# miguelmartin75/txt2vid

Hardware: AMD Instinct MI355X
Metric: TGANv2 GAN train throughput (G+D steps x global batch), 16x64x64 videos/sec (higher is better)
Workload: dtype f32; 1 GPU; BASELINE configs[1]: unconditional TGANv2 16x64x64x1, per-GPU batch 32, fp32, RSGAN + GP 0.5, Adam 2e-4 (0.5,0.999), 1 D + 1 G step, subsample_input pyramid 8/16/32/64; global_batch=32, per_gpu_batch=32, parallelism=dp1

## Files before the change

include/t2v_hip.h:

```cpp
#ifndef T2V_HIP_H
#define T2V_HIP_H

#include <stdint.h>

#ifdef __cplusplus
extern "C" {
#endif

#define T2V_OK 0
#define T2V_EINVAL (-1)
#define T2V_ELAUNCH (-2)

#define T2V_MAX_TAPS 27

typedef struct {
    int32_t N, Cin, D, H, W, Cout;
    int32_t ntaps;
    int8_t dz[T2V_MAX_TAPS], dy[T2V_MAX_TAPS], dx[T2V_MAX_TAPS];
    int8_t pad_[3];
} t2v_conv_geom;

#define T2V_MAX_GROUPS 8
typedef struct {
    const float* x;
    float* y;
    const float* mask;
    int32_t N, D, H, W;
    int32_t ntaps;
    int32_t dstride;
    int32_t ydstride;
    int32_t yoff, Dy;
    int8_t dz[T2V_MAX_TAPS], dy[T2V_MAX_TAPS], dx[T2V_MAX_TAPS], widx[T2V_MAX_TAPS];
} t2v_conv_group;

#define T2V_CONV_BIAS 1
#define T2V_CONV_RELU_IN 2
#define T2V_CONV_ACCUM 4
#define T2V_CONV_ACCUM_BIAS 16
#define T2V_CONV_BF16 32
#define T2V_CONV_MASK_OUT 8

int t2v_pack_weight(const float* w, float* wp, int Cout, int Cin, int T, const int32_t* taps, int ntaps,
                    int mode, void* stream);

int t2v_pack_weight_into(const float* w, float* wp, int Cout, int Cin, int T, const int32_t* taps, int ntaps,
                         int mode, int dst_rows, int dst_cols, int row_off, int col_off, void* stream);

typedef struct {
    const float* src;
    float* dst;
    int32_t Cout, Cin, T, ntaps, mode, dst_rows, dst_cols, row_off, col_off;
    int32_t block_begin;
    int32_t bx, by;
    int8_t taps[T2V_MAX_TAPS];
    int8_t pad_[5];
} t2v_pack_job;
int t2v_pack_job_bytes(void);
int t2v_pack_multi(const void* table , int njobs, int total_blocks, void* stream);

int t2v_conv_fwd(const float* x, const float* wp, const float* bias, float* y, float* ws, const t2v_conv_geom* g,
                 int flags, void* stream);
int64_t t2v_conv_fwd_ws_floats(const t2v_conv_geom* g);

int64_t t2v_conv_wgrad_slab_floats(const t2v_conv_geom* g, int T);
int t2v_conv_wgrad(const float* x, const float* gy, float* dw, float* slab, const t2v_conv_geom* g,
                   const int32_t* taps, int T, int flags, void* stream);

int64_t t2v_conv_fwd_grouped_ws_floats(const t2v_conv_group* groups, int ngroups, int Cin, int Cout);
int t2v_conv_fwd_grouped(const t2v_conv_group* groups, int ngroups, int Cin, int Cout, const float* wp,
                         const float* bias, float* ws, int flags, void* stream);
int64_t t2v_conv_wgrad_grouped_slab_floats(const t2v_conv_group* groups, int ngroups, int Cin, int Cout, int kD,
                                           int kH, int kW);
int t2v_conv_wgrad_grouped(const t2v_conv_group* groups, int ngroups, int Cin, int Cout, int kD, int kH, int kW,
                           float* dw, float* slab, int flags, void* stream);
#define T2V_WGRAD_MAX_SRC 6
typedef struct {
    const float* slab;
    const float* bias_slab;
    int32_t ntaps, S;
    int8_t map[T2V_MAX_TAPS];
    int8_t pad_[5];
    int64_t tap_stride;
    int64_t split_stride;
} t2v_wgrad_src;
typedef struct {
    float* dw;
    float* dbias;
    int64_t CoCi;
    int32_t T, Cout, nsrc;
    int32_t accum, accum_bias;
    int32_t kind;
    int32_t block_begin, nblocks;
    int32_t tap_major;
    int32_t pad_;
    t2v_wgrad_src src[T2V_WGRAD_MAX_SRC];
} t2v_wgrad_dest;
int t2v_conv_wgrad_grouped_partial(const t2v_conv_group* groups, int ngroups, int Cin, int Cout, int kD, int kH, int kW,
                                   float* slab, int want_bias, int flags, t2v_wgrad_src* out_src, void* stream);
int t2v_wgrad_dest_bytes(void);
int t2v_wgrad_reduce_multi(const void* table , int ndest, int total_blocks, void* stream);

int t2v_conv_fwd_plan(const t2v_conv_group* groups, int ngroups, int Cin, int Cout, int flags, int32_t* out);
int t2v_conv_wgrad_plan(const t2v_conv_group* groups, int ngroups, int Cin, int Cout, int kD, int kH, int kW, int32_t* out);
int64_t t2v_conv_wgrad_grouped_bias_slab_floats(const t2v_conv_group* groups, int ngroups, int Cin, int Cout, int kD,
                                                int kH, int kW);
int t2v_conv_wgrad_grouped_bias(const t2v_conv_group* groups, int ngroups, int Cin, int Cout, int kD, int kH, int kW,
                                float* dw, float* dbias, float* slab, int flags, void* stream);

int t2v_pack_weight_bf16(const float* w, void* wpb, int Cout, int Cin, int T, const int32_t* taps, int ntaps, int mode, void* stream);
int t2v_conv_fwd_grouped_bf16_ok(const t2v_conv_group* groups, int ngroups, int Cin, int Cout);
// ... 314 lines not shown
```

txt2vid_amd/_lib.py:

```python
import ctypes as C
import os

_HERE = os.path.dirname(os.path.abspath(__file__))
LIB_PATH = os.environ.get('T2V_LIB') or os.path.join(_HERE, 'csrc', 'libt2v_hip.so')

MAX_TAPS = 27


class ConvGeom(C.Structure):
    _fields_ = [('N', C.c_int32), ('Cin', C.c_int32), ('D', C.c_int32), ('H', C.c_int32), ('W', C.c_int32),
                ('Cout', C.c_int32), ('ntaps', C.c_int32),
                ('dz', C.c_int8 * MAX_TAPS), ('dy', C.c_int8 * MAX_TAPS), ('dx', C.c_int8 * MAX_TAPS),
                ('pad_', C.c_int8 * 3)]


class ConvGroup(C.Structure):
    _fields_ = [('x', C.c_void_p), ('y', C.c_void_p), ('mask', C.c_void_p), ('N', C.c_int32), ('D', C.c_int32), ('H', C.c_int32), ('W', C.c_int32),
                ('ntaps', C.c_int32), ('dstride', C.c_int32), ('ydstride', C.c_int32), ('yoff', C.c_int32), ('Dy', C.c_int32),
                ('dz', C.c_int8 * MAX_TAPS), ('dy', C.c_int8 * MAX_TAPS), ('dx', C.c_int8 * MAX_TAPS), ('widx', C.c_int8 * MAX_TAPS)]


class AdamJob(C.Structure):
    _fields_ = [('p', C.c_void_p), ('g', C.c_void_p), ('m', C.c_void_p), ('v', C.c_void_p), ('n', C.c_int64)]

# ... 34 lines not shown


WGRAD_MAX_SRC = 6


class WgradSrc(C.Structure):
    _fields_ = [('slab', C.c_void_p), ('bias_slab', C.c_void_p), ('ntaps', C.c_int32), ('S', C.c_int32),
                ('map', C.c_int8 * MAX_TAPS), ('pad_', C.c_int8 * 5), ('tap_stride', C.c_int64), ('split_stride', C.c_int64)]


class WgradDest(C.Structure):
    _fields_ = [('dw', C.c_void_p), ('dbias', C.c_void_p), ('CoCi', C.c_int64), ('T', C.c_int32), ('Cout', C.c_int32),
                ('nsrc', C.c_int32), ('accum', C.c_int32), ('accum_bias', C.c_int32), ('kind', C.c_int32),
                ('block_begin', C.c_int32), ('nblocks', C.c_int32), ('tap_major', C.c_int32), ('pad_', C.c_int32),
                ('src', WgradSrc * WGRAD_MAX_SRC)]


class AugMember(C.Structure):
    _fields_ = [('x', C.c_void_p), ('y', C.c_void_p), ('u', C.c_void_p), ('N', C.c_int32), ('C', C.c_int32), ('T', C.c_int32),
                ('S', C.c_int32), ('row_stride', C.c_int32), ('rows', C.c_int32), ('policy', C.c_int32), ('reserved', C.c_int32)]


class AdaLevel(C.Structure):
    _fields_ = [('real', C.c_void_p), ('fake', C.c_void_p), ('count', C.c_int32), ('reserved', C.c_int32)]


class LecamGrad(C.Structure):
    _fields_ = [('real', C.c_void_p), ('fake', C.c_void_p), ('d_real', C.c_void_p), ('d_fake', C.c_void_p), ('count', C.c_int32),
                ('reserved', C.c_int32)]


class ProjMember(C.Structure):
    _fields_ = [('g', C.c_void_p), ('f', C.c_void_p), ('s', C.c_void_p), ('base', C.c_void_p), ('out', C.c_void_p), ('b', C.c_int32),
                ('reserved', C.c_int32)]


class MbstdMember(C.Structure):
    _fields_ = [('f', C.c_void_p), ('g', C.c_void_p * 2), ('base', C.c_void_p * 2), ('gam', C.c_void_p), ('y', C.c_void_p * 2),
                ('stat', C.c_void_p), ('out', C.c_void_p), ('b', C.c_int32), ('seg', C.c_int32)]


MAX_GROUPS = 8
_P = C.c_void_p
_I = C.c_int
_L = C.c_int64
_F = C.c_float
_I3 = C.POINTER(C.c_int32)
_G = C.POINTER(ConvGeom)

SIGNATURES = {
    't2v_pack_weight': [_P, _P, _I, _I, _I, _I3, _I, _I, _P],
    't2v_pack_job_bytes': [],
    't2v_pack_multi': [_P, _I, _I, _P],
    't2v_pack_weight_into': [_P, _P, _I, _I, _I, _I3, _I, _I, _I, _I, _I, _I, _P],
    't2v_conv_fwd': [_P, _P, _P, _P, _P, _G, _I, _P],
    't2v_conv_fwd_ws_floats': [_G],
    't2v_conv_wgrad_slab_floats': [_G, _I],
    't2v_conv_fwd_grouped_ws_floats': [_P, _I, _I, _I],
    't2v_conv_fwd_grouped': [_P, _I, _I, _I, _P, _P, _P, _I, _P],
    't2v_conv_wgrad_grouped_slab_floats': [_P, _I, _I, _I, _I, _I, _I],
    't2v_conv_fwd_plan': [_P, _I, _I, _I, _I, _I3],
    't2v_nonlocal_ok': [_I, _I],
    't2v_nonlocal_fwd': [_P, _P, _P, _P, _P, _I, _I, _I, _I, _I, _P],
    't2v_nonlocal_bwd': [_P, _P, _P, _P, _P, _P, _P, _P, _P, _P, _I, _I, _I, _I, _I, _P],
    't2v_conv_wgrad_grouped_partial': [_P, _I, _I, _I, _I, _I, _I, _P, _I, _I, _P, _P],
    't2v_wgrad_dest_bytes': [],
    't2v_wgrad_reduce_multi': [_P, _I, _I, _P],
    't2v_conv_wgrad_plan': [_P, _I, _I, _I, _I, _I, _I, _I3],
    't2v_pack_weight_bf16': [_P, _P, _I, _I, _I, _P, _I, _I, _P],
    't2v_conv_fwd_grouped_bf16_ok': [_P, _I, _I, _I],
    't2v_conv_fwd_bf16_plan': [_P, _I, _I, _I, _I, _I3],
    't2v_conv_fwd_grouped_bf16': [_P, _I, _I, _I, _P, _P, _P, _I, _P],
    't2v_conv_wgrad_grouped': [_P, _I, _I, _I, _I, _I, _I, _P, _P, _I, _P],
    't2v_conv_wgrad_grouped_bias_slab_floats': [_P, _I, _I, _I, _I, _I, _I],
    't2v_conv_wgrad_grouped_bias': [_P, _I, _I, _I, _I, _I, _I, _P, _P, _P, _I, _P],
    't2v_conv_wgrad': [_P, _P, _P, _P, _G, _I3, _I, _I, _P],
    't2v_channel_sum_ws_floats': [_I, _I, _L],
    't2v_channel_sum': [_P, _P, _P, _I, _I, _L, _I, _P],
    't2v_channel_sum_grouped_ws_floats': [_P, _I, _I],
    't2v_channel_sum_grouped': [_P, _I, _I, _P, _P, _I, _P],
    't2v_relu': [_P, _P, _L, _P],
    't2v_relu_mask': [_P, _P, _P, _L, _P],
    't2v_add': [_P, _P, _P, _L, _P],
    't2v_axpby': [_F, _P, _F, _P, _P, _L, _P],
    't2v_fill': [_P, _F, _L, _P],
    't2v_tanh': [_P, _P, _L, _P],
    't2v_tanh_bwd': [_P, _P, _P, _L, _P],
    't2v_avgpool3d': [_P, _P, _P, _I, _I, _I, _I, _I, _I, _I, _I3, _I3, _I3, _P],
    't2v_avgpool3d_bwd': [_P, _P, _I, _I, _I, _I, _I, _I, _I, _I3, _I3, _I3, _P],
    't2v_avgpool3d_multi': [_P, _I, _P],
    't2v_avgpool3d_bwd_multi': [_P, _I, _P],
    't2v_rowsum': [_P, _P, _L, _L, _P],
    't2v_rowbcast': [_P, _P, _L, _L, _P],
    't2v_upsample2x': [_P, _P, _L, _I, _I, _P],
    't2v_upsample2x_bwd': [_P, _P, _L, _I, _I, _P],
    't2v_upsample2x_add': [_P, _P, _P, _L, _I, _I, _P],
    't2v_rsgan_mean_multi': [_P, _I, _P, _P],
    't2v_rsgan_mean_multi_bwd': [_P, _I, _P, _P],
    't2v_bn_ws_floats': [_I, _I, _L],
    't2v_bn_plan': [_I, _I, _L, _I3],
    't2v_bn_stats': [_P, _P, _P, _P, _P, _I, _I, _L, _F, _F, _P],
    't2v_bn_apply': [_P, _P, _P, _P, _P, _I, _I, _L, _I, _P],
    't2v_bn_bwd': [_P, _P, _P, _P, _P, _P, _P, _P, _P, _I, _I, _L, _I, _P],
    't2v_bn_train_fwd': [_P, _P, _P, _P, _P, _P, _P, _P, _I, _I, _L, _F, _F, _I, _P, _P],
    't2v_bn_train_bwd': [_P, _P, _P, _P, _P, _P, _P, _P, _P, _I, _I, _L, _I, _P],
    't2v_bn_train_fwd_up': [_P, _P, _P, _P, _P, _P, _P, _P, _I, _I, _I, _I, _F, _F, _I, _P, _P],
# ... 134 lines not shown
```

txt2vid_amd/csrc/conv.hip:

```cpp
#include <hip/hip_runtime.h>
#include <stdint.h>
#include "../../include/t2v_hip.h"

typedef float f32x16 __attribute__((ext_vector_type(16)));

#ifdef T2V_STAMPS
__device__ unsigned long long* g_stamps = nullptr;
__device__ unsigned int g_stamps_cap = 0;
extern "C" int t2v_stamps_set(void* buf, unsigned int cap_records) {
    if (hipMemcpyToSymbol(HIP_SYMBOL(g_stamps), &buf, sizeof(buf)) != hipSuccess) return -1;
    if (hipMemcpyToSymbol(HIP_SYMBOL(g_stamps_cap), &cap_records, sizeof(cap_records)) != hipSuccess) return -1;
    return 0;
}
__device__ __forceinline__ unsigned long long stamp_now() {
    unsigned long long t;
    __builtin_amdgcn_sched_barrier(0);
    asm volatile("s_memtime %0\n\ts_waitcnt lgkmcnt(0)" : "=s"(t) :: "memory");
    __builtin_amdgcn_sched_barrier(0);
    return t;
}
#define STAMP(v) const unsigned long long v = stamp_now()
#define STAMP_ACC(acc, a, b) acc += (b) - (a)
#else
#define STAMP(v)
// ... 48 lines not shown
            g_prof_cur = r;
        }
    }
    ~ProfScope() { g_prof_cur = nullptr; }
    static void set_plan(const int32_t* plan, int n) {
        if (g_prof_cur) for (int i = 0; i < n && i < 8; ++i) g_prof_cur->plan[i] = plan[i];
    }
};
#define T2V_LAUNCH_PROF(kernel, grid, block, shm, stream, ...) do {                                                      \
        (void)hipGetLastError();                                                                                          \
        if (g_prof_cur) {                                                                                                 \
            ProfRec* r_ = g_prof_cur; g_prof_cur = nullptr;                                                               \
            hipExtLaunchKernelGGL(kernel, grid, block, shm, stream, r_->e0, r_->e1, 0, __VA_ARGS__);                      \
        } else hipLaunchKernelGGL(kernel, grid, block, shm, stream, __VA_ARGS__);                                         \
    } while (0)

extern "C" int t2v_prof_begin(int max_records) {
    if (max_records < 1 || max_records > (1 << 20)) return T2V_EINVAL;
    if ((int)g_prof.recs.size() < max_records) {
        size_t old = g_prof.recs.size();
        g_prof.recs.resize(max_records);
        for (size_t i = old; i < g_prof.recs.size(); ++i) {
            if (hipEventCreate(&g_prof.recs[i].e0) != hipSuccess || hipEventCreate(&g_prof.recs[i].e1) != hipSuccess) return T2V_ELAUNCH;
        }
    }
    g_prof.used = 0;
    g_prof.on = true;
    return T2V_OK;
}
extern "C" int t2v_prof_end(double* out, int nkinds) {
    g_prof.on = false;
    if (!out || nkinds < 1) return T2V_EINVAL;
    for (int i = 0; i < nkinds * 3; ++i) out[i] = 0.0;
    FILE* dump = nullptr;
    if (const char* path = getenv("T2V_PROF_DUMP")) dump = fopen(path, "w");
    if (dump) fprintf(dump, "kind,flops,ms,M,Cin,Cout,taps,groups,S,plan\n");
    for (size_t i = 0; i < g_prof.used; ++i) {
        ProfRec& r = g_prof.recs[i];
        if (hipEventSynchronize(r.e1) != hipSuccess) return T2V_ELAUNCH;
        float ms = 0.f;
        if (hipEventElapsedTime(&ms, r.e0, r.e1) != hipSuccess) return T2V_ELAUNCH;
        if (r.kind >= 0 && r.kind < nkinds) { out[r.kind * 3] += ms; out[r.kind * 3 + 1] += r.flops; out[r.kind * 3 + 2] += 1.0; }
        if (dump) fprintf(dump, "%d,%.0f,%.6f,%ld,%d,%d,%d,%d,%d,%d:%d:%d:%d:%d:%d:%d:%d\n", r.kind, r.flops, ms, r.M, r.Cin, r.Cout, r.taps,
                          r.groups, r.S, r.plan[0], r.plan[1], r.plan[2], r.plan[3], r.plan[4], r.plan[5], r.plan[6], r.plan[7]);
    }
    if (dump) fclose(dump);
    int dropped = (g_prof.used >= g_prof.recs.size()) ? 1 : 0;
    g_prof.used = 0;
    return dropped;
}

struct TapList { int32_t n; int32_t t[T2V_MAX_TAPS]; };

__global__ __launch_bounds__(256) void pack_weight_kernel(const float* __restrict__ w, float* __restrict__ wp,
                                                          int Cout, int Cin, int T, TapList taps, int mode, int dst_rows,
                                                          int dst_cols, int row_off, int col_off) {
    __shared__ float tile[32][33];
    const int j = blockIdx.z;
    const bool src_tm = mode & 8;
    mode &= 7;
    const int t = mode ? (T - 1 - taps.t[j]) : taps.t[j];
    const int tx = threadIdx.x & 31, ty = threadIdx.x >> 5;
    const int co0 = blockIdx.y * 32, ci0 = blockIdx.x * 32;
    const size_t sco = src_tm ? (size_t)Cin : (size_t)Cin * T, sci = src_tm ? 1 : (size_t)T;
    const size_t st = src_tm ? (size_t)t * Cout * Cin : (size_t)t;
    if (mode == 0) {
        for (int r = ty; r < 32; r += 8) {
            int co = co0 + r, ci = ci0 + tx;
            tile[r][tx] = (co < Cout && ci < Cin) ? w[co * sco + ci * sci + st] : 0.f;
        }
        __syncthreads();
        for (int r = ty; r < 32; r += 8) {
            int ci = ci0 + r, co = co0 + tx;
            if (ci < Cin && co < Cout) wp[((size_t)j * dst_rows + row_off + ci) * dst_cols + col_off + co] = tile[tx][r];
        }
    } else {
        for (int r = ty; r < 32; r += 8) {
            int co = co0 + r, ci = ci0 + tx;
            if (co < Cout && ci < Cin)
                wp[((size_t)j * dst_rows + row_off + co) * dst_cols + col_off + ci] = w[co * sco + ci * sci + st];
        }
    }
}

extern "C" int t2v_pack_weight_into(const float* w, float* wp, int Cout, int Cin, int T, const int32_t* taps, int ntaps,
                                    int mode, int dst_rows, int dst_cols, int row_off, int col_off, void* stream) {
    if (!w || !wp || ntaps < 1 || ntaps > T2V_MAX_TAPS || T > T2V_MAX_TAPS || row_off < 0 || col_off < 0) return T2V_EINVAL;
    if ((mode & ~8) != 0 && (mode & ~8) != 1) return T2V_EINVAL;
    const int rows = (mode & 7) ? Cout : Cin, cols = (mode & 7) ? Cin : Cout;
    if (row_off + rows > dst_rows || col_off + cols > dst_cols) return T2V_EINVAL;
    TapList tl;
    tl.n = ntaps;
    for (int i = 0; i < ntaps; ++i) {
        if (taps[i] < 0 || taps[i] >= T) return T2V_EINVAL;
        tl.t[i] = taps[i];
    }
    dim3 grid((Cin + 31) / 32, (Cout + 31) / 32, ntaps);
    T2V_LAUNCH(pack_weight_kernel, grid, dim3(256), 0, (hipStream_t)stream, w, wp, Cout, Cin, T, tl, mode, dst_rows, dst_cols,
               row_off, col_off);
    return launch_status();
}

extern "C" int t2v_pack_weight(const float* w, float* wp, int Cout, int Cin, int T, const int32_t* taps, int ntaps,
                               int mode, void* stream) {
    return t2v_pack_weight_into(w, wp, Cout, Cin, T, taps, ntaps, mode, (mode & 7) ? Cout : Cin, (mode & 7) ? Cin : Cout, 0, 0, stream);
}


struct PackJob {
    const float* src;
    float* dst;
    int32_t Cout, Cin, T, ntaps, mode, dst_rows, dst_cols, row_off, col_off, block_begin, bx, by;
    int8_t taps[T2V_MAX_TAPS];
    int8_t pad_[5];
};

__global__ __launch_bounds__(256) void pack_multi_kernel(const PackJob* __restrict__ table, int njobs) {
    __shared__ float tile[32][33];
    __shared__ PackJob job;
    if (threadIdx.x == 0) {
        int lo = 0, hi = njobs - 1;
        while (lo < hi) {
            const int mid = (lo + hi + 1) >> 1;
            if (table[mid].block_begin <= (int)blockIdx.x) lo = mid; else hi = mid - 1;
        }
        job = table[lo];
    }
    __syncthreads();
    const int b = (int)blockIdx.x - job.block_begin;
    const int bxi = b % job.bx, byi = (b / job.bx) % job.by, j = b / (job.bx * job.by);
    const int Cout = job.Cout, Cin = job.Cin, T = job.T;
    const int jm = job.mode & 7;
    const bool src_tm = job.mode & 8;
    const bool mirror = jm == 1 || jm == 3, transpose = jm == 0 || jm == 3, b16 = jm >= 2;
    const int t = mirror ? (T - 1 - job.taps[j]) : job.taps[j];
    const size_t sco = src_tm ? (size_t)Cin : (size_t)Cin * T, sci = src_tm ? 1 : (size_t)T;
    const size_t st = src_tm ? (size_t)t * Cout * Cin : (size_t)t;
    const int tx = threadIdx.x & 31, ty = threadIdx.x >> 5;
    const int co0 = byi * 32, ci0 = bxi * 32;
    const float* __restrict__ w = job.src;
    float* __restrict__ wp = job.dst;
    __bf16* __restrict__ wpb = reinterpret_cast<__bf16*>(job.dst);
    if (transpose) {
        for (int r = ty; r < 32; r += 8) {
            int co = co0 + r, ci = ci0 + tx;
            tile[r][tx] = (co < Cout && ci < Cin) ? w[co * sco + ci * sci + st] : 0.f;
        }
        __syncthreads();
        for (int r = ty; r < 32; r += 8) {
            int ci = ci0 + r, co = co0 + tx;
            if (ci < Cin && co < Cout) {
                const size_t o = ((size_t)j * job.dst_rows + job.row_off + ci) * job.dst_cols + job.col_off + co;
                if (b16) wpb[o] = (__bf16)tile[tx][r]; else wp[o] = tile[tx][r];
            }
        }
    } else {
        for (int r = ty; r < 32; r += 8) {
            int co = co0 + r, ci = ci0 + tx;
            if (co < Cout && ci < Cin) {
                const size_t o = ((size_t)j * job.dst_rows + job.row_off + co) * job.dst_cols + job.col_off + ci;
                const float v = w[co * sco + ci * sci + st];
                if (b16) wpb[o] = (__bf16)v; else wp[o] = v;
            }
        }
    }
}

extern "C" int t2v_pack_job_bytes(void) { return (int)sizeof(PackJob); }

extern "C" int t2v_pack_multi(const void* table, int njobs, int total_blocks, void* stream) {
    if (!table || njobs < 1 || total_blocks < 1) return T2V_EINVAL;
    T2V_LAUNCH(pack_multi_kernel, dim3((unsigned)total_blocks), dim3(256), 0, (hipStream_t)stream, (const PackJob*)table, njobs);
    return launch_status();
}

struct GroupTable {
    t2v_conv_group g[T2V_MAX_GROUPS];
    int32_t tile_start[T2V_MAX_GROUPS + 1];
    int64_t out_start[T2V_MAX_GROUPS + 1];
    int32_t n;
};

template <int NCO, int NM, int WCO, int WM>
__device__ __forceinline__ void igemm_epilogue(f32x16 (&acc)[NCO][NM], const GroupTable& tab, const int gi, const t2v_conv_group& gd,
                                               const float* __restrict__ bias, float* __restrict__ slab, const int Cout,
                                               const int flags, const int nsplit, const int m0, const int co0, const int M,
                                               const int DHW, const int wm, const int wco, const int l31, const int hi,
                                               const int yds = 1, const int yoff = 0, const int DHWy = 0, const int HW = 1) {
    const bool split = nsplit > 1;
    const bool has_bias = !split && (flags & T2V_CONV_BIAS) && bias != nullptr;
    const bool accum = !split && (flags & T2V_CONV_ACCUM);
    const bool mask_out = !split && (flags & T2V_CONV_MASK_OUT) && gd.mask != nullptr;
    float* out = split ? slab + (size_t)blockIdx.z * (size_t)tab.out_start[tab.n] + (size_t)tab.out_start[gi] : gd.y;
#pragma unroll
    for (int j = 0; j < NM; ++j) {
        const int m = m0 + wm * WM + j * 32 + l31;
        if (m >= M) continue;
        const int n = m / DHW;
        int sp = m - n * DHW;
        int cs = DHW;
        if (yds == 2) {
            const int e = sp / HW;
            sp += (e + yoff) * HW;
            cs = DHWy;
        }
        float* py = out + (size_t)n * Cout * cs + sp;
        if (mask_out) {
            const float* pm = gd.mask + (size_t)n * Cout * cs + sp;
#pragma unroll
            for (int i = 0; i < NCO; ++i) {
                float mv[16];
#pragma unroll
                for (int r = 0; r < 16; ++r) {
                    const int co = co0 + wco * WCO + i * 32 + (r & 3) + 8 * (r >> 2) + 4 * hi;
                    mv[r] = pm[(size_t)(co < Cout ? co : Cout - 1) * cs];
                }
#pragma unroll
                for (int r = 0; r < 16; ++r) {
// ... 1605 lines not shown
#pragma unroll
        for (int g = 0; g < KPT / 8; ++g) {
            bf16x8 o;
#pragma unroll
            for (int j = 0; j < 8; ++j) o[j] = (__bf16)(ok ? fmaxf(v[g * 8 + j], relu_floor) : 0.f);
            *reinterpret_cast<bf16x8*>(dst + g * 8) = o;
        }
    };
    bf16x8 zero8;
#pragma unroll
    for (int j = 0; j < 8; ++j) zero8[j] = (__bf16)0.f;
    auto stage = [&]() {
        put_row(Xs + (1 + ma_l) * B16_KP + kq * KPT, ra, pend_av);
        if (halo_thread) put_row(Xs + (he ? BM + 1 : 0) * B16_KP + hq * KPT, rh, pend_hv);
#pragma unroll
        for (int d = 0; d < 3; ++d)
            if (d < ndx) *reinterpret_cast<bf16x8*>(Ws + d * (BN * B16_KP) + wc_l * B16_KP + wk_l) = w_ok ? rw8[d] : zero8;
    };

    if (tid < 4) *reinterpret_cast<bf16x8*>(Xs + ZROW * B16_KP + tid * 8) = zero8;
    if (q0 < q1) load_round(q0);
    for (int q = q0; q < q1; ++q) {
        stage();
        __syncthreads();
        if (q + 1 < q1) load_round(q + 1);
#pragma unroll
        for (int d = 0; d < 3; ++d) {
            if (d < ndx) {
                const int dx = ndx == 3 ? d - 1 : 0;
                const __bf16* ws = Ws + d * (BN * B16_KP) + (wco * WCO + l31) * B16_KP + 8 * hi;
                const __bf16* xs[NM];
#pragma unroll
                for (int j = 0; j < NM; ++j) {
                    const bool keep = dx < 0 ? can_l[j] : (dx > 0 ? can_r[j] : true);
                    xs[j] = Xs + (keep ? 1 + dx + wm * WM + j * 32 + l31 : ZROW) * B16_KP + 8 * hi;
                }
#pragma unroll
                for (int ks = 0; ks < BKT / 16; ++ks) {
                    const bf16x8 a = *reinterpret_cast<const bf16x8*>(ws + ks * 16);
#pragma unroll
                    for (int j = 0; j < NM; ++j) {
                        const bf16x8 b = *reinterpret_cast<const bf16x8*>(xs[j] + ks * 16);
                        acc[0][j] = __builtin_amdgcn_mfma_f32_32x32x16_bf16(a, b, acc[0][j], 0, 0, 0);
                    }
                }
            }
        }
        __syncthreads();
    }
    igemm_epilogue<NCO, NM, WCO, WM>(acc, tab, gi, gd, bias, slab, Cout, flags, nsplit, m0, co0, M, DHWo, wm, wco, l31, hi, yds, gd.yoff,
                                     gd.Dy * HW, HW);
}

__global__ void pack_weight_bf16_kernel(const float* __restrict__ w, __bf16* __restrict__ wpb, int Cout, int Cin, int T,
                                        TapList taps, int mode) {
    const int j = blockIdx.y;
    const int t = mode ? (T - 1 - taps.t[j]) : taps.t[j];
    const long n = (long)Cout * Cin;
    for (long i = (long)blockIdx.x * 256 + threadIdx.x; i < n; i += (long)gridDim.x * 256) {
        int row, k;
        if (mode == 0) { row = (int)(i / Cin); k = (int)(i - (long)row * Cin); wpb[(size_t)j * n + i] = (__bf16)w[((size_t)row * Cin + k) * T + t]; }
        else { row = (int)(i / Cout); k = (int)(i - (long)row * Cout); wpb[(size_t)j * n + i] = (__bf16)w[((size_t)k * Cin + row) * T + t]; }
    }
}
extern "C" int t2v_pack_weight_bf16(const float* w, void* wpb, int Cout, int Cin, int T, const int32_t* taps, int ntaps, int mode,
                                    void* stream) {
    if (!w || !wpb || !taps || Cout < 1 || Cin < 1 || T < 1 || ntaps < 1 || ntaps > T2V_MAX_TAPS) return T2V_EINVAL;
    TapList tl;
    tl.n = ntaps;
    for (int i = 0; i < T2V_MAX_TAPS; ++i) tl.t[i] = i < ntaps ? taps[i] : 0;
    long nb = ((long)Cout * Cin + 255) / 256;
    if (nb > 1024) nb = 1024;
    T2V_LAUNCH(pack_weight_bf16_kernel, dim3((unsigned)nb, (unsigned)ntaps), dim3(256), 0, (hipStream_t)stream, w, (__bf16*)wpb, Cout, Cin,
               T, tl, mode);
    return launch_status();
}

__global__ __launch_bounds__(256) void splitk_reduce_kernel(const GroupTable tab, const float* __restrict__ slab,
                                                            const float* __restrict__ bias, int S, int Cout, int flags) {
    const bool has_bias = (flags & T2V_CONV_BIAS) && bias != nullptr;
    const bool accum = flags & T2V_CONV_ACCUM;
    const long total = tab.out_start[tab.n];
    for (long i = (long)blockIdx.x * 256 + threadIdx.x; i < total; i += (long)gridDim.x * 256) {
        int gi = 0;
#pragma unroll
        for (int k = 1; k < T2V_MAX_GROUPS; ++k)
            if (k < tab.n && i >= tab.out_start[k]) gi = k;
        const long li = i - tab.out_start[gi];
        float v = 0.f;
#pragma unroll 8
        for (int s = 0; s < S; ++s) v += slab[(size_t)s * total + i];
        if (has_bias) {
            const int DHW = tab.g[gi].D * tab.g[gi].H * tab.g[gi].W;
            v += bias[(li / DHW) % Cout];
        }
        float* y = tab.g[gi].y;
        if ((flags & T2V_CONV_MASK_OUT) && tab.g[gi].mask) v = tab.g[gi].mask[li] > 0.f ? v : 0.f;
        y[li] = accum ? y[li] + v : v;
    }
}


#define THIN_MAX_W 16384

template <int NC>
__global__ __launch_bounds__(256) void conv_thin_kernel(const GroupTable tab, const float* __restrict__ wp,
                                                        const float* __restrict__ bias, const int Cin, const int Cout,
                                                        const int nslots, const int flags) {
    __shared__ float sw[THIN_MAX_W];
    __shared__ int s_off[T2V_MAX_TAPS];
    __shared__ int s_widx[T2V_MAX_TAPS];
    const int tid = threadIdx.x;
    int gi = 0;
#pragma unroll
    for (int k = 1; k < T2V_MAX_GROUPS; ++k)
        if (k < tab.n && (int)blockIdx.x >= tab.tile_start[k]) gi = k;
    const t2v_conv_group& gd = tab.g[gi];
    const int D = gd.D, H = gd.H, W = gd.W, HW = H * W, DHW = D * HW;
    const int M = gd.N * DHW;
    const int ntaps = gd.ntaps;
    for (int i = tid; i < nslots * Cin * Cout; i += 256) sw[i] = wp[i];
    __shared__ int s_d3[T2V_MAX_TAPS];
    if (tid < ntaps) {
        const int dz = gd.dz[tid], dy = gd.dy[tid], dx = gd.dx[tid];
        s_off[tid] = dz * HW + dy * W + dx;
        s_d3[tid] = (dz + 1) | ((dy + 1) << 2) | ((dx + 1) << 4);
        s_widx[tid] = gd.widx[tid];
// ... 2978 lines not shown
```

txt2vid_amd/functional.py:

```python
import contextlib
import ctypes as C
import os
import weakref

import torch
from torch.autograd import Function
from torch.autograd.function import once_differentiable

from ._lib import lib, check, ConvGeom, ConvGroup, PackJob, WgradSrc, WgradDest, WGRAD_MAX_SRC, MAX_TAPS, MAX_GROUPS

FLAG_BIAS, FLAG_RELU_IN, FLAG_ACCUM, FLAG_MASK_OUT, FLAG_ACCUM_BIAS, FLAG_BF16 = 1, 2, 4, 8, 16, 32


from ._ops import _stream, _p, _c


def tap_major(w):
    nd = w.dim()
    fwd = tuple(range(2, nd)) + (0, 1)
    back = tuple(range(nd - 2, nd)) + tuple(range(nd - 2))
    return w.permute(*fwd).contiguous().permute(*back)


def is_tap_major(w):
# ... 336 lines not shown

def set_conv_precision(p):
    global CONV_PRECISION
    if p not in ('fp32', 'bf16'):
        raise ValueError(p)
    old, CONV_PRECISION = CONV_PRECISION, p
    return old


def packed_weight_bf16(w5, ts, mode):
    Cout, Cin = w5.shape[0], w5.shape[1]
    base = w5._base if w5._base is not None else w5

    def pack(dst):
        check(lib().t2v_pack_weight_bf16(_p(w5), _p(dst), Cout, Cin, ts.T, ts.taps_c, len(ts.taps), mode, _stream()),
              't2v_pack_weight_bf16')
    if not isinstance(base, torch.nn.Parameter):
        wp = torch.empty((len(ts.taps), Cin * Cout), device=w5.device, dtype=torch.bfloat16)
        pack(wp)
        return wp
    key = ('bf16', tuple(w5.shape), ts.mask, mode)
    tag = _wtag(base, w5.data_ptr())
    ent = _pack_cache.setdefault(id(base), {})
    hit = ent.get(key)
    if hit is not None and hit[0]() is base:
        if hit[1] != tag:
            pack(hit[2])
            hit[1] = tag
        return hit[2]
    wp = torch.empty((len(ts.taps), Cin * Cout), device=w5.device, dtype=torch.bfloat16)
    pack(wp)
    ent[key] = [weakref.ref(base), tag, wp, ts]
    return wp


_repack_tables = {}


def _pack_job_of(p, key, hit):
    if callable(hit[3]):
        return hit[4]
    if key[0] == 'bf16':
        _, shape5, _, mode = key
        ts = hit[3]
        Cout, Cin = shape5[0], shape5[1]
        src = p if tuple(p.shape) == tuple(shape5) else p.view(shape5)
        return (src, hit[2], Cout, Cin, ts.T, list(ts.taps), 2 + mode, (Cin if mode else Cout), (Cout if mode else Cin), 0, 0)
    shape5, _, mode = key
    geom = hit[3]
    Cout, Cin = shape5[0], shape5[1]
    return (p, hit[2], Cout, Cin, geom.T, list(geom.taps), mode, (Cout if mode else Cin), (Cin if mode else Cout), 0, 0)


def repack_params(params):
    params = list(params)
    jobs = []
    for p in params:
        ent = _pack_cache.get(id(p))
        if not ent:
            continue
        for key, hit in ent.items():
            if hit[0]() is p:
                jobs.append((p, key, hit))
    if not jobs:
        return
    sig = tuple((id(p), key, hit[2].data_ptr(), p.data_ptr()) for p, key, hit in jobs)
    tkey = tuple(id(p) for p in params)
    tab = _repack_tables.get(tkey)
    if tab is None or tab[0] != sig:
        assert C.sizeof(PackJob) == lib().t2v_pack_job_bytes()
        arr = (PackJob * len(jobs))()
        blocks = 0
        for a, (p, key, hit) in zip(arr, jobs):
            src, dst, Cout, Cin, T, taps, mode, rows, cols, ro, co = _pack_job_of(p, key, hit)
            a.src, a.dst = src.data_ptr(), dst.data_ptr()
            a.Cout, a.Cin, a.T, a.ntaps, a.mode = Cout, Cin, T, len(taps), mode
            a.dst_rows, a.dst_cols, a.row_off, a.col_off = rows, cols, ro, co
            a.bx, a.by = (Cin + 31) // 32, (Cout + 31) // 32
            a.block_begin = blocks
            for j, t in enumerate(taps):
                a.taps[j] = t
            blocks += a.bx * a.by * len(taps)
        host = torch.frombuffer(bytearray(bytes(arr)), dtype=torch.uint8).clone()
        dev = host.to(params[0].device)
        tab = (sig, dev, len(jobs), blocks)
        _repack_tables[tkey] = tab
    check(lib().t2v_pack_multi(_p(tab[1]), tab[2], tab[3], _stream()), 't2v_pack_multi')
    for p, key, hit in jobs:
        hit[1] = _wtag(p)
    for fkey, fh in _fused_cache.items():
        if any(r() is p for r in fh[0] for p in params):
            fh[1] = tuple(_wtag(w()) for w in fh[0] if w() is not None)


_fused_cache = {}


def packed_fused(ws, ts, mode):
    n = len(ws)
    Cout, Cin = ws[0].shape[0], ws[0].shape[1]
    bases = [w._base if w._base is not None else w for w in ws]
    cacheable = all(isinstance(b_, torch.nn.Parameter) for b_ in bases)
    key = (tuple(id(b_) for b_ in bases), tuple(ws[0].shape), ts.mask, mode)
    hit = _fused_cache.get(key) if cacheable else None
    if hit is not None and all(r() is b_ for r, b_ in zip(hit[0], bases)):
        tag = tuple(_wtag(b_, w.data_ptr()) for b_, w in zip(bases, ws))
        if hit[1] != tag:
            for i, w in enumerate(ws):
                hit[3][i](w)
            hit[1] = tag
        return hit[2]
    rows, cols = (Cin, n * Cout) if mode == 0 else (n * Cout, Cin)
    wp = torch.empty((len(ts.taps), rows * cols), device=ws[0].device, dtype=torch.float32)
    refresh = []
    for i, w in enumerate(ws):
        ro, co = (0, i * Cout) if mode == 0 else (i * Cout, 0)

        tm = 8 if is_tap_major(w) else 0

        def fn(wi, ro=ro, co=co, tm=tm):
            check(lib().t2v_pack_weight_into(_p(wi), _p(wp), Cout, Cin, ts.T, ts.taps_c, len(ts.taps), mode | tm, rows, cols,
                                             ro, co, _stream()), 't2v_pack_weight_into')
        refresh.append(fn)
        fn(w)
        if cacheable:
            _pack_cache.setdefault(id(bases[i]), {})[('fused', key, i)] = [weakref.ref(bases[i]), _wtag(bases[i], w.data_ptr()), wp, fn,
                                                                           (w, wp, Cout, Cin, ts.T, list(ts.taps), mode | tm, rows, cols, ro, co)]
    if cacheable:
        _fused_cache[key] = [[weakref.ref(b_) for b_ in bases], tuple(_wtag(b_, w.data_ptr()) for b_, w in zip(bases, ws)), wp, refresh]
    return wp


def conv_packed_raw(x5, wp, cin, cout, k, bias=None, out=None, accum=False):
    x5 = _c(x5)
    y = out if out is not None else torch.empty((x5.shape[0], cout) + tuple(x5.shape[2:]), device=x5.device, dtype=torch.float32)
# ... 2059 lines not shown
```

Baseline: 3043 videos/s.

## Coalesce weight packing by reading tap groups of source rows into LDS

Weight-packing kernels now give each block a group of up to 9 consecutive temporal taps for a 32x32 channel tile. The block loads that contiguous slice of the non-tap-major source into LDS with coalesced reads, then writes every tap that falls in the group. Before, each block read a single strided tap per element. The bf16 pack path is also moved onto the same unified tiled kernel. The goal is less strided, uncoalesced global traffic when repacking weights after every optimizer step. The cost is more LDS use, extra synchronisation, and a more complex block-to-job mapping that the Python table builder must match.

Measured after the change: 3075 videos/s (median of 6 runs). 1.1% higher.

```diff
diff --git a/include/t2v_hip.h b/include/t2v_hip.h
--- a/include/t2v_hip.h
+++ b/include/t2v_hip.h
@@ -56,6 +56,7 @@
     int8_t pad_[5];
 } t2v_pack_job;
 int t2v_pack_job_bytes(void);
+int t2v_pack_job_groups(int T, int ntaps, int mode);
 int t2v_pack_multi(const void* table , int njobs, int total_blocks, void* stream);
 
 int t2v_conv_fwd(const float* x, const float* wp, const float* bias, float* y, float* ws, const t2v_conv_geom* g,
diff --git a/txt2vid_amd/_lib.py b/txt2vid_amd/_lib.py
--- a/txt2vid_amd/_lib.py
+++ b/txt2vid_amd/_lib.py
@@ -110,6 +110,7 @@
     't2v_pack_weight': [_P, _P, _I, _I, _I, _I3, _I, _I, _P],
     't2v_pack_job_bytes': [],
     't2v_pack_multi': [_P, _I, _I, _P],
+    't2v_pack_job_groups': [_I, _I, _I],
     't2v_pack_weight_into': [_P, _P, _I, _I, _I, _I3, _I, _I, _I, _I, _I, _I, _P],
     't2v_conv_fwd': [_P, _P, _P, _P, _P, _G, _I, _P],
     't2v_conv_fwd_ws_floats': [_G],
diff --git a/txt2vid_amd/csrc/conv.hip b/txt2vid_amd/csrc/conv.hip
--- a/txt2vid_amd/csrc/conv.hip
+++ b/txt2vid_amd/csrc/conv.hip
@@ -124,35 +124,124 @@
 
 struct TapList { int32_t n; int32_t t[T2V_MAX_TAPS]; };
 
-__global__ __launch_bounds__(256) void pack_weight_kernel(const float* __restrict__ w, float* __restrict__ wp,
+#define PK_TG 9
+#define PK_CW 16
+#define PK_PITCH (PK_CW * PK_TG + 1)
+__host__ __device__ inline int pack_job_groups(int T, int ntaps, int mode) {
+    return ((mode & 8) || T <= PK_TG) ? ntaps : (T + PK_TG - 1) / PK_TG;
+}
+extern "C" int t2v_pack_job_groups(int T, int ntaps, int mode) {
+    if (T < 1 || ntaps < 1) return T2V_EINVAL;
+    return pack_job_groups(T, ntaps, mode);
+}
+
+#define T2V_GLOBAL __attribute__((address_space(1)))
+__device__ __forceinline__ float gload(const float* p) { return *(const T2V_GLOBAL float*)p; }
+__device__ __forceinline__ void pack_store(void* __restrict__ dst, size_t o, float v, bool b16) {
+    if (b16) ((T2V_GLOBAL __bf16*)dst)[o] = (__bf16)v; else ((T2V_GLOBAL float*)dst)[o] = v;
+}
+
+template <int NT>
+__device__ __forceinline__ void pack_group_read(float* __restrict__ lds, const float* __restrict__ w, int Cout, int Cin, int T,
+                                                int co0, int ci0, int t0, int nt_rt) {
+    const int nt = NT ? NT : nt_rt;
+    const int per_row = PK_CW * nt, total = 32 * per_row;
+    const float* __restrict__ base = w + ((size_t)co0 * Cin + ci0) * T + t0;
+    const int rmax = Cout - 1 - co0, cmax = Cin - 1 - ci0;
+#pragma unroll 3
+    for (int e = threadIdx.x; e < total; e += 256) {
+        const int r = e / per_row, q = e - r * per_row;
+        const int ci_l = q / nt, tt = q - ci_l * nt;
+        lds[r * PK_PITCH + q] = gload(base + (unsigned)((min(r, rmax) * Cin + min(ci_l, cmax)) * T + tt));
+    }
+}
+
+template <class TapT>
+__device__ __forceinline__ void pack_tile(float* __restrict__ lds, const float* __restrict__ w, void* __restrict__ dst, const int Cout,
+                                          const int Cin, const int T, const int ntaps, const TapT* taps, const int mode,
+                                          const int dst_rows, const int dst_cols, const int row_off, const int col_off, const int bxi,
+                                          const int byi, const int z) {
+    const int jm = mode & 7;
+    const bool src_tm = mode & 8;
+    const bool mirror = jm == 1 || jm == 3, transpose = jm == 0 || jm == 3, b16 = jm >= 2;
+    const int tx = threadIdx.x & 31, ty = threadIdx.x >> 5;
+    const int co0 = byi * 32, ci0 = bxi * 32;
+    int j1 = z;
+    if (!src_tm && T > PK_TG) {
+        const int t0 = z * PK_TG, nt = T - t0 < PK_TG ? T - t0 : PK_TG;
+        int nl = 0;
+        for (int j = 0; j < ntaps; ++j) {
+            const int tj = __builtin_amdgcn_readfirstlane((int)taps[j]);
+            const int tt = (mirror ? T - 1 - tj : tj) - t0;
+            if (tt >= 0 && tt < nt) { ++nl; j1 = j; }
+        }
+        if (nl == 0) return;
+        if (nl > 1) {
+            for (int cih = ci0; cih < ci0 + 32 && cih < Cin; cih += PK_CW) {
+                if (cih != ci0) __syncthreads();
+                if (nt == 9) pack_group_read<9>(lds, w, Cout, Cin, T, co0, cih, t0, nt);
+                else pack_group_read<0>(lds, w, Cout, Cin, T, co0, cih, t0, nt);
+                __syncthreads();
+                for (int j = 0; j < ntaps; ++j) {
+                    const int tj = __builtin_amdgcn_readfirstlane((int)taps[j]);
+                    const int tt = (mirror ? T - 1 - tj : tj) - t0;
+                    if (tt < 0 || tt >= nt) continue;
+                    const size_t ob = (size_t)j * dst_rows + row_off;
+                    if (transpose) {
+#pragma unroll
+                        for (int r = ty; r < PK_CW; r += 8) {
+                            const int ci = cih + r, co = co0 + tx;
+                            if (ci < Cin && co < Cout) pack_store(dst, (ob + ci) * dst_cols + col_off + co, lds[tx * PK_PITCH + r * nt + tt], b16);
+                        }
+                    } else {
+#pragma unroll
+                        for (int r = ty * 2 + (tx >> 4); r < 32; r += 16) {
+                            const int co = co0 + r, cl = tx & 15, ci = cih + cl;
+                            if (co < Cout && ci < Cin) pack_store(dst, (ob + co) * dst_cols + col_off + ci, lds[r * PK_PITCH + cl * nt + tt], b16);
+                        }
+                    }
+                }
+            }
+            return;
+        }
+    }
+    const int j = j1;
+    const int tj = __builtin_amdgcn_readfirstlane((int)taps[j]);
+    const int t = mirror ? (T - 1 - tj) : tj;
+    const size_t sco = src_tm ? (size_t)Cin : (size_t)Cin * T, sci = src_tm ? 1 : (size_t)T;
+    const size_t st = src_tm ? (size_t)t * Cout * Cin : (size_t)t;
+    const size_t ob = (size_t)j * dst_rows + row_off;
+    if (transpose) {
+#pragma unroll
+        for (int r = ty; r < 32; r += 8) {
+            const int co = min(co0 + r, Cout - 1), ci = min(ci0 + tx, Cin - 1);
+            lds[r * 33 + tx] = gload(w + co * sco + ci * sci + st);
+        }
+        __syncthreads();
+#pragma unroll
+        for (int r = ty; r < 32; r += 8) {
+            const int ci = ci0 + r, co = co0 + tx;
+            if (ci < Cin && co < Cout) pack_store(dst, (ob + ci) * dst_cols + col_off + co, lds[tx * 33 + r], b16);
+        }
+    } else {
+#pragma unroll
+        for (int r = ty; r < 32; r += 8) {
+            const int co = co0 + r, ci = ci0 + tx;
+            if (co < Cout && ci < Cin) pack_store(dst, (ob + co) * dst_cols + col_off + ci, gload(w + co * sco + ci * sci + st), b16);
+        }
+    }
+}
+
+__global__ __launch_bounds__(256) void pack_weight_kernel(const float* __restrict__ w, void* __restrict__ wp,
                                                           int Cout, int Cin, int T, TapList taps, int mode, int dst_rows,
                                                           int dst_cols, int row_off, int col_off) {
-    __shared__ float tile[32][33];
-    const int j = blockIdx.z;
-    const bool src_tm = mode & 8;
-    mode &= 7;
-    const int t = mode ? (T - 1 - taps.t[j]) : taps.t[j];
-    const int tx = threadIdx.x & 31, ty = threadIdx.x >> 5;
-    const int co0 = blockIdx.y * 32, ci0 = blockIdx.x * 32;
-    const size_t sco = src_tm ? (size_t)Cin : (size_t)Cin * T, sci = src_tm ? 1 : (size_t)T;
-    const size_t st = src_tm ? (size_t)t * Cout * Cin : (size_t)t;
-    if (mode == 0) {
-        for (int r = ty; r < 32; r += 8) {
-            int co = co0 + r, ci = ci0 + tx;
-            tile[r][tx] = (co < Cout && ci < Cin) ? w[co * sco + ci * sci + st] : 0.f;
-        }
-        __syncthreads();
-        for (int r = ty; r < 32; r += 8) {
-            int ci = ci0 + r, co = co0 + tx;
-            if (ci < Cin && co < Cout) wp[((size_t)j * dst_rows + row_off + ci) * dst_cols + col_off + co] = tile[tx][r];
-        }
-    } else {
-        for (int r = ty; r < 32; r += 8) {
-            int co = co0 + r, ci = ci0 + tx;
-            if (co < Cout && ci < Cin)
-                wp[((size_t)j * dst_rows + row_off + co) * dst_cols + col_off + ci] = w[co * sco + ci * sci + st];
-        }
-    }
+    __shared__ float lds[32 * PK_PITCH];
+    __shared__ int s_taps[T2V_MAX_TAPS];
+    if ((int)threadIdx.x < taps.n) s_taps[threadIdx.x] = taps.t[threadIdx.x];
+    __syncthreads();
+    const int bx = (Cin + 31) / 32, by = (Cout + 31) / 32;
+    const int b = blockIdx.x;
+    pack_tile(lds, w, wp, Cout, Cin, T, taps.n, s_taps, mode, dst_rows, dst_cols, row_off, col_off, b % bx, (b / bx) % by, b / (bx * by));
 }
 
 extern "C" int t2v_pack_weight_into(const float* w, float* wp, int Cout, int Cin, int T, const int32_t* taps, int ntaps,
@@ -167,9 +256,10 @@
         if (taps[i] < 0 || taps[i] >= T) return T2V_EINVAL;
         tl.t[i] = taps[i];
     }
-    dim3 grid((Cin + 31) / 32, (Cout + 31) / 32, ntaps);
-    T2V_LAUNCH(pack_weight_kernel, grid, dim3(256), 0, (hipStream_t)stream, w, wp, Cout, Cin, T, tl, mode, dst_rows, dst_cols,
-               row_off, col_off);
+    const long nb = (long)((Cin + 31) / 32) * ((Cout + 31) / 32) * pack_job_groups(T, ntaps, mode);
+    if (nb > 0x7fffffffL) return T2V_EINVAL;
+    T2V_LAUNCH(pack_weight_kernel, dim3((unsigned)nb), dim3(256), 0, (hipStream_t)stream, w, (void*)wp, Cout, Cin, T, tl, mode, dst_rows,
+               dst_cols, row_off, col_off);
     return launch_status();
 }
 
@@ -188,7 +278,7 @@
 };
 
 __global__ __launch_bounds__(256) void pack_multi_kernel(const PackJob* __restrict__ table, int njobs) {
-    __shared__ float tile[32][33];
+    __shared__ float lds[32 * PK_PITCH];
     __shared__ PackJob job;
     if (threadIdx.x == 0) {
         int lo = 0, hi = njobs - 1;
@@ -199,43 +289,12 @@
         job = table[lo];
     }
     __syncthreads();
-    const int b = (int)blockIdx.x - job.block_begin;
-    const int bxi = b % job.bx, byi = (b / job.bx) % job.by, j = b / (job.bx * job.by);
-    const int Cout = job.Cout, Cin = job.Cin, T = job.T;
-    const int jm = job.mode & 7;
-    const bool src_tm = job.mode & 8;
-    const bool mirror = jm == 1 || jm == 3, transpose = jm == 0 || jm == 3, b16 = jm >= 2;
-    const int t = mirror ? (T - 1 - job.taps[j]) : job.taps[j];
-    const size_t sco = src_tm ? (size_t)Cin : (size_t)Cin * T, sci = src_tm ? 1 : (size_t)T;
-    const size_t st = src_tm ? (size_t)t * Cout * Cin : (size_t)t;
-    const int tx = threadIdx.x & 31, ty = threadIdx.x >> 5;
-    const int co0 = byi * 32, ci0 = bxi * 32;
-    const float* __restrict__ w = job.src;
-    float* __restrict__ wp = job.dst;
-    __bf16* __restrict__ wpb = reinterpret_cast<__bf16*>(job.dst);
-    if (transpose) {
-        for (int r = ty; r < 32; r += 8) {
-            int co = co0 + r, ci = ci0 + tx;
-            tile[r][tx] = (co < Cout && ci < Cin) ? w[co * sco + ci * sci + st] : 0.f;
-        }
-        __syncthreads();
-        for (int r = ty; r < 32; r += 8) {
-            int ci = ci0 + r, co = co0 + tx;
-            if (ci < Cin && co < Cout) {
-                const size_t o = ((size_t)j * job.dst_rows + job.row_off + ci) * job.dst_cols + job.col_off + co;
-                if (b16) wpb[o] = (__bf16)tile[tx][r]; else wp[o] = tile[tx][r];
-            }
-        }
-    } else {
-        for (int r = ty; r < 32; r += 8) {
-            int co = co0 + r, ci = ci0 + tx;
-            if (co < Cout && ci < Cin) {
-                const size_t o = ((size_t)j * job.dst_rows + job.row_off + co) * job.dst_cols + job.col_off + ci;
-                const float v = w[co * sco + ci * sci + st];
-                if (b16) wpb[o] = (__bf16)v; else wp[o] = v;
-            }
-        }
-    }
+    const int b = (int)blockIdx.x - __builtin_amdgcn_readfirstlane(job.block_begin);
+    const int bx = __builtin_amdgcn_readfirstlane(job.bx), by = __builtin_amdgcn_readfirstlane(job.by);
+    const int bxi = b % bx, byi = (b / bx) % by, z = b / (bx * by);
+    pack_tile(lds, job.src, job.dst, __builtin_amdgcn_readfirstlane(job.Cout), __builtin_amdgcn_readfirstlane(job.Cin),
+              __builtin_amdgcn_readfirstlane(job.T), __builtin_amdgcn_readfirstlane(job.ntaps), job.taps,
+              __builtin_amdgcn_readfirstlane(job.mode), job.dst_rows, job.dst_cols, job.row_off, job.col_off, bxi, byi, z);
 }
 
 extern "C" int t2v_pack_job_bytes(void) { return (int)sizeof(PackJob); }
@@ -1947,27 +2006,17 @@
                                      gd.Dy * HW, HW);
 }
 
-__global__ void pack_weight_bf16_kernel(const float* __restrict__ w, __bf16* __restrict__ wpb, int Cout, int Cin, int T,
-                                        TapList taps, int mode) {
-    const int j = blockIdx.y;
-    const int t = mode ? (T - 1 - taps.t[j]) : taps.t[j];
-    const long n = (long)Cout * Cin;
-    for (long i = (long)blockIdx.x * 256 + threadIdx.x; i < n; i += (long)gridDim.x * 256) {
-        int row, k;
-        if (mode == 0) { row = (int)(i / Cin); k = (int)(i - (long)row * Cin); wpb[(size_t)j * n + i] = (__bf16)w[((size_t)row * Cin + k) * T + t]; }
-        else { row = (int)(i / Cout); k = (int)(i - (long)row * Cout); wpb[(size_t)j * n + i] = (__bf16)w[((size_t)k * Cin + row) * T + t]; }
-    }
-}
 extern "C" int t2v_pack_weight_bf16(const float* w, void* wpb, int Cout, int Cin, int T, const int32_t* taps, int ntaps, int mode,
                                     void* stream) {
     if (!w || !wpb || !taps || Cout < 1 || Cin < 1 || T < 1 || ntaps < 1 || ntaps > T2V_MAX_TAPS) return T2V_EINVAL;
+    mode = mode ? 1 : 0;
     TapList tl;
     tl.n = ntaps;
     for (int i = 0; i < T2V_MAX_TAPS; ++i) tl.t[i] = i < ntaps ? taps[i] : 0;
-    long nb = ((long)Cout * Cin + 255) / 256;
-    if (nb > 1024) nb = 1024;
-    T2V_LAUNCH(pack_weight_bf16_kernel, dim3((unsigned)nb, (unsigned)ntaps), dim3(256), 0, (hipStream_t)stream, w, (__bf16*)wpb, Cout, Cin,
-               T, tl, mode);
+    const long nb = (long)((Cin + 31) / 32) * ((Cout + 31) / 32) * pack_job_groups(T, ntaps, 2 + mode);
+    if (nb > 0x7fffffffL) return T2V_EINVAL;
+    T2V_LAUNCH(pack_weight_kernel, dim3((unsigned)nb), dim3(256), 0, (hipStream_t)stream, w, wpb, Cout, Cin, T, tl, 2 + mode,
+               mode ? Cin : Cout, mode ? Cout : Cin, 0, 0);
     return launch_status();
 }
 
diff --git a/txt2vid_amd/functional.py b/txt2vid_amd/functional.py
--- a/txt2vid_amd/functional.py
+++ b/txt2vid_amd/functional.py
@@ -412,6 +412,13 @@
     return (p, hit[2], Cout, Cin, geom.T, list(geom.taps), mode, (Cout if mode else Cin), (Cin if mode else Cout), 0, 0)
 
 
+def pack_job_groups(T, ntaps, mode):
+    n = lib().t2v_pack_job_groups(T, ntaps, mode)
+    if n < 1:
+        raise ValueError('t2v_pack_job_groups(%d, %d, %d) = %d' % (T, ntaps, mode, n))
+    return n
+
+
 def repack_params(params):
     params = list(params)
     jobs = []
@@ -440,7 +447,7 @@
             a.block_begin = blocks
             for j, t in enumerate(taps):
                 a.taps[j] = t
-            blocks += a.bx * a.by * len(taps)
+            blocks += a.bx * a.by * pack_job_groups(T, len(taps), mode)
         host = torch.frombuffer(bytearray(bytes(arr)), dtype=torch.uint8).clone()
         dev = host.to(params[0].device)
         tab = (sig, dev, len(jobs), blocks)
```
